# luchsonice/3dod

Hardware: AMD Instinct MI355X
Metric: images/sec Cube R-CNN DLA34-FPN train step (higher is better)
Workload: dtype fp32; 1 GPU; Cube R-CNN DLA34+FPN train step (fwd+loss+bwd+allreduce+SGD), 4 img/GPU 512x512, Base_Omni3D.yaml semantics (BASELINE configs[3] per-GPU shard); global_batch=4, parallelism=dp1, weight_gradient_reduce=pixel splits stored and added in a fixed order (CR_DETERMINISTIC=1), valid=True

## Files before the change

### 3dod_amd/_lib.py

```python
import ctypes
import os
import threading

import torch

_HERE = os.path.dirname(os.path.abspath(__file__))
LIB_PATH = os.path.join(_HERE, "lib", "libcr3dod.so")

c_void_p, c_int, c_int64, c_float = ctypes.c_void_p, ctypes.c_int, ctypes.c_int64, ctypes.c_float
P = c_void_p

SIGNATURES = {
    "cr_ctx_create": [c_int, P, ctypes.POINTER(P)],
    "cr_ctx_destroy": [P],
    "cr_ctx_set_stream": [P, P],
    "cr_abi_version": [],
    "cr_cuboid_corners": [P, P, P, c_int64, P],
    "cr_cubes_project_score": [P, P, c_int64, c_int64, P, c_int, c_float, c_float, P, P, P, P,
                               P, P, P, P, P, P, P, P, P],
    "cr_cubes_project_score_fast": [P, P, c_int64, c_int64, P, c_int, c_float, c_float, P, P, P, P,
                                    P, P, P, P, P, P, P, P, P, P],
    "cr_propose": [P, P, c_int64, P, c_int, c_int, P, P, P, c_int64, P, c_int, P, P, P, P, P],
    "cr_ransac_plane": [P, P, c_int64, P, c_int64, c_float, P, P, P],
    "cr_ransac_plane_batched": [P, P, P, c_int, c_int64, P, c_int64, c_float, P, P, P],
# ... 43 lines not shown
    "cr_conv2d_grouped_bwd_weight": [P, P, P, P, P, c_int, c_int, c_int, c_int, c_int, c_int, c_int, c_int, c_int, c_int, c_int,
                                     P, c_int64],
    "cr_cast_f32_to_bf16": [P, P, P, c_int64],
    "cr_weight_transpose": [P, P, P, c_int, c_int, c_int, c_int],
    "cr_colsum_accum": [P, P, c_int, c_int64, c_int, P, P],
    "cr_bn_fwd": [P, P, P, c_int, P, P, P, P, c_int64, c_int, c_int, c_float, c_float, P, P, P, c_int],
    "cr_bn_bwd": [P, P, P, P, P, P, P, P, P, P, P, c_int64, c_int, c_int, c_int],
    "cr_bn_bwd_mask": [P, P, P, P, P, P, P, P, P, P, P, P, c_int64, c_int, c_int, c_int],
    "cr_bn_frozen_unfold": [P, P, P, P, P, P, P, c_float, P, c_int, P, P, c_int, c_int],
    "cr_pool2x_fwd": [P, P, P, c_int, c_int, c_int, c_int, c_int, c_int],
    "cr_pool2x_bwd": [P, P, P, P, c_int, c_int, c_int, c_int, c_int, c_int, P],
    "cr_upsample2x_add": [P, P, P, P, c_int, c_int, c_int, c_int, c_int],
    "cr_sum2x2": [P, P, P, c_int, c_int, c_int, c_int, c_int],
    "cr_preprocess": [P, P, P, c_int, c_int, c_int, P, P, c_int],
    "cr_roi_align_fwd": [P, P, P, P, P, c_int, c_int, P, c_int64, c_int, c_int, P, c_int],
    "cr_roi_align_bwd": [P, P, P, P, P, c_int, c_int, P, c_int64, c_int, c_int, P, c_int],
    "cr_conv2d_fwd_group": [P, c_int, P, P, P, P, P, P, c_int, c_int, c_int, c_int, P, P, c_int, c_int],
    "cr_wino_filter": [P, P, P, c_int, c_int, c_int],
    "cr_gemm_batched_f32": [P, P, P, P, c_int, c_int, c_int, c_int, c_int64, c_int64, c_int64],
    "cr_wino_input": [P, c_int, P, P, P, P, c_int, P, c_int64],
    "cr_wino_output": [P, c_int, P, P, P, P, P, c_int, c_int64, P, c_int, P],
    "cr_wino_dy": [P, c_int, P, P, P, P, c_int, P, c_int64, P],
    "cr_wino_filter_grad": [P, P, P, c_int, c_int, P, P],
    "cr_wgrad_batched_f32": [P, P, P, P, c_int, c_int, c_int, c_int, c_int64, c_int64, c_int64],
    "cr_conv2d_bwd_data_group": [P, c_int, P, P, P, P, P, P, c_int, c_int, c_int, c_int, c_int, P],
    "cr_conv2d_bwd_weight_group": [P, c_int, P, P, P, P, P, P, P, c_int, c_int, c_int, c_int, c_int],
    "cr_conv2d_bwd_weight_multi": [P, c_int, P, P, P, P, P, P, P, P, P, P, P, P, c_int],
    "cr_roi_align_bwd_set": [P, P, P, P, P, c_int, c_int, c_int, P, c_int64, c_int, c_int, P, c_int],
    "cr_roi_pool_fwd": [P, P, P, P, P, c_int, c_int, c_int, P, c_int64, c_int, c_int, c_int, c_int, P, P, c_int],
    "cr_roi_pool_bwd": [P, P, P, P, P, c_int, c_int, c_int, P, c_int64, c_int, c_int, c_int, c_int, P, P, c_int],
    "cr_roi_pool_bwd_set": [P, P, P, P, P, c_int, c_int, c_int, P, c_int64, c_int, c_int, c_int, c_int, P, c_int],
    "cr_nms_grouped": [P, P, P, c_int, c_int, c_float, P, P],
    "cr_cube_loss_fwd": [P, P, c_int64, c_int, c_int, c_int, c_int, P, P],
    "cr_cube_loss_bwd": [P, P, c_int64, c_int, c_int, c_int, c_int, P, P, P, P, P, P],
    "cr_rpn_decode_select": [P, P, P, P, P, c_int, c_int, c_int, P, c_float, P, c_float, P, P, P],
    "cr_box_match": [P, P, c_int, P, P, c_int, c_int, c_int, P, P, P, P],
    "cr_rpn_label": [P, P, P, P, P, P, P, c_int, c_int, c_int, c_float, c_float, P, c_float, P, P, P, P],
    "cr_rpn_scatter": [P, P, P, c_int, P, P, c_int, c_int, P, c_float, c_int, c_int, P],
    "cr_rpn_loss": [P, P, P, P, P, P, P, c_int, c_int, c_int, P, P, P, P, P],
    "cr_rpn_loss_opt": [P, P, P, P, P, P, P, c_int, c_int, c_int, P, c_int, c_int, c_float, c_float, P, P, P, P],
    "cr_roi_label": [P, P, P, P, P, P, P, c_int, c_int, c_int, c_int, c_float, c_float, c_float, P, P, P],
    "cr_roi_compact": [P, P, P, c_int, P, P, c_int, c_int, P, P, P, c_int, c_int, P, P, P, P, P],
    "cr_box_loss": [P, P, P, P, P, P, P, P, c_int, c_int, c_int, c_int, P, c_float, P, P, P, P, P],
    "cr_box_loss_opt": [P, P, P, P, P, P, P, P, c_int, c_int, c_int, c_int, P, c_float, c_float, c_int, P, P, P, P, P],
    "cr_det_scores": [P, P, c_int, P, c_int, P, P, c_int, c_int, c_int, c_int, c_float, P, P],
    "cr_det_gather": [P, P, P, P, c_int, P, P, c_int, c_int, c_int, c_int, c_int, P, c_float, P, P, P, P],
# ... 165 lines not shown
```

### 3dod_amd/csrc/winograd.hip

```cpp
#include "cr_common.h"

#define WINO_MAX_MAPS 8
struct WinoMap { const float* src; float* dst; const float* acc; int N, H, W, tbase, blk0; };
struct WinoGeo { WinoMap m[WINO_MAX_MAPS]; int n, C, T; };

__device__ __forceinline__ int wino_find(const WinoGeo& g, int blk) {
    int i = 0;
    while (i + 1 < g.n && blk >= g.m[i + 1].blk0) ++i;
    return i;
}

typedef float vf1 __attribute__((ext_vector_type(1)));
typedef float vf2 __attribute__((ext_vector_type(2)));
typedef float vf4 __attribute__((ext_vector_type(4)));
#define WINO_TPB 8
#define WINO_TPB_DY 16
#define WINO_DB_SLOTS 16

struct WinoTile { int n, ty, tx, c; bool ok; };
template <int VEC>
__device__ __forceinline__ WinoTile wino_tile(const WinoGeo& g, const WinoMap& m, int tile_in_block, int tpb) {
    const int cgs = g.C / (64 * VEC);
    const int local = (int)blockIdx.x - m.blk0;
    const int cg = local % cgs, chunk = local / cgs;
// ... 59 lines not shown
            for (int e = 0; e < VEC; ++e) b[e] = bias[w.c + e];
        }
        const float* o = M + ((size_t)m.tbase + ((size_t)w.n * th + w.ty) * tw + w.tx) * C + w.c;
        VT q[4][4];
#pragma unroll
        for (int i = 0; i < 4; ++i)
#pragma unroll
            for (int j = 0; j < 4; ++j) q[i][j] = *(const VT*)(o + (i * 4 + j) * plane);
        VT s[2][4];
#pragma unroll
        for (int j = 0; j < 4; ++j) { s[0][j] = (q[0][j] + q[1][j]) + q[2][j]; s[1][j] = (q[1][j] - q[2][j]) - q[3][j]; }
#pragma unroll
        for (int i = 0; i < 2; ++i) {
            VT y0 = (s[i][0] + s[i][1]) + s[i][2] + b, y1 = (s[i][1] - s[i][2]) - s[i][3] + b;
            const size_t p = (((size_t)w.n * m.H + 2 * w.ty + i) * m.W + 2 * w.tx) * C + w.c;
            if (relu) { y0 = __builtin_elementwise_max(y0, (VT)(0.f)); y1 = __builtin_elementwise_max(y1, (VT)(0.f)); }
            if (m.acc) { y0 += *(const VT*)(m.acc + p); y1 += *(const VT*)(m.acc + p + C); }
            *(VT*)(m.dst + p) = y0;
            *(VT*)(m.dst + p + C) = y1;
        }
    }
}

__global__ __launch_bounds__(256) void k_wino_filter(const float* __restrict__ w, float* __restrict__ U, int O, int C, int mode) {
    const int idx = blockIdx.x * 256 + threadIdx.x;
    if (idx >= O * C) return;
    const int o = idx / C, c = idx - o * C;
    float g[3][3];
#pragma unroll
    for (int r = 0; r < 3; ++r)
#pragma unroll
        for (int s = 0; s < 3; ++s) g[r][s] = w[((size_t)(o * 3 + (mode ? 2 - r : r)) * 3 + (mode ? 2 - s : s)) * C + c];
    float t[4][3];
#pragma unroll
    for (int s = 0; s < 3; ++s) {
        t[0][s] = g[0][s];
        t[1][s] = 0.5f * ((g[0][s] + g[1][s]) + g[2][s]);
        t[2][s] = 0.5f * ((g[0][s] - g[1][s]) + g[2][s]);
        t[3][s] = g[2][s];
    }
    const size_t plane = (size_t)O * C;
    const size_t at = mode ? (size_t)c * O + o : (size_t)o * C + c;
#pragma unroll
    for (int i = 0; i < 4; ++i) {
        U[(i * 4 + 0) * plane + at] = t[i][0];
        U[(i * 4 + 1) * plane + at] = 0.5f * ((t[i][0] + t[i][1]) + t[i][2]);
        U[(i * 4 + 2) * plane + at] = 0.5f * ((t[i][0] - t[i][1]) + t[i][2]);
        U[(i * 4 + 3) * plane + at] = t[i][2];
    }
}

template <typename VT>
__global__ __launch_bounds__(256) void k_wino_dy(WinoGeo g, float* __restrict__ dM, float* __restrict__ db) {
    constexpr int VEC = sizeof(VT) / 4;
    __shared__ VT s_sum[4][64];
    const WinoMap& m = g.m[wino_find(g, (int)blockIdx.x)];
    const int C = g.C, th = m.H >> 1, tw = m.W >> 1;
    const int lane = threadIdx.x & 63, wave = threadIdx.x >> 6;
    const size_t plane = (size_t)g.T * C;
    VT acc = (VT)(0.f);
    int c = wino_tile<VEC>(g, m, 0, WINO_TPB_DY).c;
    for (int k = wave; k < WINO_TPB_DY; k += 4) {
        const WinoTile w = wino_tile<VEC>(g, m, k, WINO_TPB_DY);
        if (!w.ok) break;
        const float* p = m.src + (((size_t)w.n * m.H + 2 * w.ty) * m.W + 2 * w.tx) * C + w.c;
        const VT d00 = *(const VT*)p, d01 = *(const VT*)(p + C), d10 = *(const VT*)(p + (size_t)m.W * C),
                 d11 = *(const VT*)(p + (size_t)m.W * C + C);
        acc += (d00 + d01) + (d10 + d11);
        const VT t[4][2] = {{d00, d01}, {d00 + d10, d01 + d11}, {d00 - d10, d01 - d11}, {-d10, -d11}};
        float* o = dM + ((size_t)m.tbase + ((size_t)w.n * th + w.ty) * tw + w.tx) * C + w.c;
#pragma unroll
        for (int i = 0; i < 4; ++i) {
            *(VT*)(o + (i * 4 + 0) * plane) = t[i][0];
            *(VT*)(o + (i * 4 + 1) * plane) = t[i][0] + t[i][1];
            *(VT*)(o + (i * 4 + 2) * plane) = t[i][0] - t[i][1];
            *(VT*)(o + (i * 4 + 3) * plane) = -t[i][1];
        }
    }
    if (db) {
        s_sum[wave][lane] = acc;
        __syncthreads();
        if (wave == 0) {
            const VT v = (s_sum[0][lane] + s_sum[1][lane]) + (s_sum[2][lane] + s_sum[3][lane]);
#pragma unroll
            for (int e = 0; e < VEC; ++e) atomicAdd(db + (size_t)(blockIdx.x % WINO_DB_SLOTS) * C + c + e, v[e]);
        }
    }
}

__global__ __launch_bounds__(256) void k_wino_filter_grad(const float* __restrict__ dU, float* __restrict__ dw, int O, int C,
                                                          const float* __restrict__ db_part, float* __restrict__ db) {
    const int idx = blockIdx.x * 256 + threadIdx.x;
    if (idx >= O * C) return;
    const int o = idx / C, c = idx - o * C;
    if (db && c == 0) {
        float sum = 0.f;
        for (int k = 0; k < WINO_DB_SLOTS; ++k) sum += db_part[(size_t)k * O + o];
        db[o] += sum;
    }
    const size_t plane = (size_t)O * C;
    float u[4][4];
#pragma unroll
    for (int i = 0; i < 4; ++i)
#pragma unroll
        for (int j = 0; j < 4; ++j) u[i][j] = dU[(i * 4 + j) * plane + idx];
    float t[3][4];
#pragma unroll
    for (int j = 0; j < 4; ++j) {
        t[0][j] = u[0][j] + 0.5f * (u[1][j] + u[2][j]);
        t[1][j] = 0.5f * (u[1][j] - u[2][j]);
        t[2][j] = 0.5f * (u[1][j] + u[2][j]) + u[3][j];
    }
// ... 10 lines not shown
static int wino_geo(const char* who, WinoGeo& g, int n, const float* const* srcs, float* const* dsts, const float* const* accs,
                    const int* Ns, const int* Hs, const int* Ws, int C, int64_t T, int tpb, unsigned* blocks, int* vec) {
    CR_CHECK_ARG(n >= 1 && n <= WINO_MAX_MAPS, "%s: 1..%d maps", who, WINO_MAX_MAPS);
    CR_CHECK_ARG(C > 0 && C % 64 == 0, "%s: channels %% 64", who);
    g.n = n; g.C = C; g.T = (int)T;
    const int v = C % 256 == 0 ? 4 : C % 128 == 0 ? 2 : 1;
    *vec = v;
    int tb = 0, blk = 0;
    for (int i = 0; i < n; ++i) {
        CR_CHECK_ARG(Ns[i] > 0 && Hs[i] > 0 && Ws[i] > 0 && Hs[i] % 2 == 0 && Ws[i] % 2 == 0, "%s: map %d needs even H and W", who, i);
        g.m[i].src = srcs ? srcs[i] : nullptr; g.m[i].dst = dsts ? dsts[i] : nullptr; g.m[i].acc = accs ? accs[i] : nullptr;
        g.m[i].N = Ns[i]; g.m[i].H = Hs[i]; g.m[i].W = Ws[i]; g.m[i].tbase = tb; g.m[i].blk0 = blk;
        tb += Ns[i] * (Hs[i] / 2) * (Ws[i] / 2);
        blk += (int)cr_cdiv((int64_t)Ns[i] * (Hs[i] / 2) * (Ws[i] / 2), tpb) * (C / (64 * v));
    }
    CR_CHECK_ARG(tb == T && (int64_t)T * C * 16 < (1ll << 40), "%s: T = %lld does not match the maps (%d tiles)", who, (long long)T, tb);
    for (int i = n; i < WINO_MAX_MAPS; ++i) g.m[i] = g.m[n - 1];
    *blocks = (unsigned)blk;
    return CR_OK;
}

extern "C" int cr_wino_filter(cr_ctx* ctx, const float* w_krsc, float* U, int O, int C, int backward) {
    CR_CHECK_ARG(ctx && w_krsc && U && O > 0 && C > 0, "cr_wino_filter: bad args");
    hipLaunchKernelGGL(k_wino_filter, dim3((unsigned)cr_cdiv((int64_t)O * C, 256)), dim3(256), 0, ctx->stream, w_krsc, U, O, C, backward ? 1 : 0);
    CR_LAUNCH_CHECK();
    return CR_OK;
}

extern "C" int cr_wino_input(cr_ctx* ctx, int n, const float* const* xs, const int* Ns, const int* Hs, const int* Ws, int C,
                             float* V, int64_t T) {
    CR_CHECK_ARG(ctx && xs && Ns && Hs && Ws && V, "cr_wino_input: NULL pointer");
    WinoGeo g;
    unsigned blocks = 0;
    int vec = 1;
    int rc = wino_geo("cr_wino_input", g, n, xs, nullptr, nullptr, Ns, Hs, Ws, C, T, WINO_TPB, &blocks, &vec);
    if (rc) return rc;
    if (vec == 4) hipLaunchKernelGGL(k_wino_input<vf4>, dim3(blocks), dim3(256), 0, ctx->stream, g, V);
    else if (vec == 2) hipLaunchKernelGGL(k_wino_input<vf2>, dim3(blocks), dim3(256), 0, ctx->stream, g, V);
    else hipLaunchKernelGGL(k_wino_input<vf1>, dim3(blocks), dim3(256), 0, ctx->stream, g, V);
    CR_LAUNCH_CHECK();
    return CR_OK;
}

extern "C" int cr_wino_output(cr_ctx* ctx, int n, const float* M, float* const* ys, const int* Ns, const int* Hs, const int* Ws,
                              int O, int64_t T, const float* bias, int relu, const float* const* accs) {
    CR_CHECK_ARG(ctx && M && ys && Ns && Hs && Ws, "cr_wino_output: NULL pointer");
    WinoGeo g;
// ... 3 lines not shown
    if (rc) return rc;
    if (vec == 4) hipLaunchKernelGGL(k_wino_output<vf4>, dim3(blocks), dim3(256), 0, ctx->stream, g, M, bias, relu);
    else if (vec == 2) hipLaunchKernelGGL(k_wino_output<vf2>, dim3(blocks), dim3(256), 0, ctx->stream, g, M, bias, relu);
    else hipLaunchKernelGGL(k_wino_output<vf1>, dim3(blocks), dim3(256), 0, ctx->stream, g, M, bias, relu);
    CR_LAUNCH_CHECK();
    return CR_OK;
}

extern "C" int cr_wino_dy(cr_ctx* ctx, int n, const float* const* dys, const int* Ns, const int* Hs, const int* Ws, int O,
                          float* dM, int64_t T, float* db) {
    CR_CHECK_ARG(ctx && dys && Ns && Hs && Ws && dM, "cr_wino_dy: NULL pointer");
    WinoGeo g;
    unsigned blocks = 0;
    int vec = 1;
    int rc = wino_geo("cr_wino_dy", g, n, dys, nullptr, nullptr, Ns, Hs, Ws, O, T, WINO_TPB_DY, &blocks, &vec);
    if (rc) return rc;
    if (vec == 4) hipLaunchKernelGGL(k_wino_dy<vf4>, dim3(blocks), dim3(256), 0, ctx->stream, g, dM, db);
    else if (vec == 2) hipLaunchKernelGGL(k_wino_dy<vf2>, dim3(blocks), dim3(256), 0, ctx->stream, g, dM, db);
    else hipLaunchKernelGGL(k_wino_dy<vf1>, dim3(blocks), dim3(256), 0, ctx->stream, g, dM, db);
    CR_LAUNCH_CHECK();
    return CR_OK;
}

extern "C" int cr_wino_filter_grad(cr_ctx* ctx, const float* dU, float* dw, int O, int C, const float* db_part, float* db) {
    CR_CHECK_ARG(ctx && dU && dw && O > 0 && C > 0 && (!db == !db_part), "cr_wino_filter_grad: bad args");
    hipLaunchKernelGGL(k_wino_filter_grad, dim3((unsigned)cr_cdiv((int64_t)O * C, 256)), dim3(256), 0, ctx->stream, dU, dw, O, C,
                       db_part, db);
    CR_LAUNCH_CHECK();
    return CR_OK;
}
```

### 3dod_amd/cubercnn/modeling/graphed.py

```python
import contextlib
import gc

import torch
import torch.nn as nn

from ... import hipops as ops


@contextlib.contextmanager
def capture_guard():
    was = gc.isenabled()
    gc.collect()
    _empty_graveyard()
    gc.disable()
    keep, prev = [], ops._PLAN_KEEP[0]
    ops._PLAN_KEEP[0] = keep
    try:
        yield keep
    finally:
        ops._PLAN_KEEP[0] = prev
        if was:
            gc.enable()
        _empty_graveyard()

# ... 29 lines not shown
    dev = None

    def __del__(self):
        try:
            _bury_or_drain(self)
        except Exception:
            pass


@contextlib.contextmanager
def _fresh_leaves(modules):
    swapped = []
    for mod in modules:
        for m in mod.modules():
            for name, p in list(m._parameters.items()):
                if p is None:
                    continue
                q = nn.Parameter(p.data, requires_grad=p.requires_grad)
                sink = ops.grad_sink(p)
                if sink is not None:
                    q._cr_grad = sink
                if hasattr(p, "_cr_bank"):
                    q._cr_bank = p._cr_bank
                m._parameters[name] = q
                swapped.append((m, name, p))
    try:
        yield
    finally:
        for m, name, p in swapped:
            m._parameters[name] = p


class _Replay(torch.autograd.Function):
    @staticmethod
    def forward(ctx, runner, trigger):
        runner.fwd_graph.replay()
        ctx.runner = runner
        ctx.set_materialize_grads(False)
        return tuple(o.detach() for o in runner.static_outs)

    @staticmethod
    def backward(ctx, *grads):
        r = ctx.runner
        if r.pre_bwd is not None:
            r.pre_bwd()
        for sg, g in zip(r.static_grads, grads):
            if g is None:
                sg.zero_()
            elif g.data_ptr() != sg.data_ptr():
                sg.copy_(g)
        r.bwd_graph.replay()
        if r.bwd_graph2 is not None:
# ... 195 lines not shown
```

### 3dod_amd/hipops.py

```python
import contextlib
import ctypes
import math
import os

import torch

from . import _lib

bf16 = torch.bfloat16
f32 = torch.float32
STAT_REPL = 32

_PRECISIONS = {"fp32": (f32, 1), "f32": (f32, 1), "float32": (f32, 1), "fp32x3": (f32, 2), "bf16": (bf16, 0),
               "bfloat16": (bf16, 0)}
_ACT = [_PRECISIONS[os.environ.get("CR_PRECISION", "fp32").lower()]]


def set_precision(name):
    prev = precision()
    _ACT[0] = _PRECISIONS[str(name).lower()]
    return prev


def precision():
# ... 1022 lines not shown

def wino_supported(xs, weight, k, pad):
    return (winograd_on() and k == 3 and pad == 1 and xs[0].dtype == f32 and _ACT[0][1] == 1 and len(xs) <= 8
            and weight.shape[0] % 128 == 0 and weight.shape[1] % 128 == 0
            and all(x.shape[1] % 2 == 0 and x.shape[2] % 2 == 0 for x in xs))


WINO_MIN_TILES = int(os.environ.get("CR_WINO_MIN_TILES", "4096"))


def _wino_plan(xs, ws, bs, k, pad):
    n = len(xs)
    if not wino_supported(xs, ws[0], k, pad):
        return [False] * n
    if all(w is ws[0] for w in ws) and all(b is bs[0] for b in bs):
        return "shared"
    return [x.shape[0] * (x.shape[1] // 2) * (x.shape[2] // 2) >= WINO_MIN_TILES for x in xs]


def wino_gemm_raw(V, U, M, T, cin, cout):
    _lib.call("cr_gemm_batched_f32", V, U, M, T, cin, cout, 16, T * cin, cout * cin, T * cout)


def wino_conv3x3_group(srcs, w_krsc, dsts, bias, relu, accs, backward, keep_v=False):
    cast = lambda a: ctypes.cast(a, ctypes.c_void_p)
    assert w_krsc.dim() == 4 and w_krsc.shape[2:] == (3, 3) and w_krsc.is_contiguous(memory_format=torch.channels_last)
    O, C = w_krsc.shape[0], w_krsc.shape[1]
    cin, cout = (O, C) if backward else (C, O)
    dev = srcs[0].device
    T = sum(x.shape[0] * (x.shape[1] // 2) * (x.shape[2] // 2) for x in srcs)
    V, M, U = _wino_buffers(T, cin, cout, dev)
    U = U[:16 * O * C]
    if keep_v:
        V = torch.empty((16, T, cin), dtype=f32, device=dev)
    _lib.call("cr_wino_filter", w_krsc, U, O, C, int(backward))
    Ns, Hs, Ws = _int_table([x.shape[0] for x in srcs]), _int_table([x.shape[1] for x in srcs]), _int_table([x.shape[2] for x in srcs])
    _lib.call("cr_wino_input", len(srcs), cast(_ptr_table(srcs)), cast(Ns), cast(Hs), cast(Ws), cin, V, T)
    wino_gemm_raw(V, U, M, T, cin, cout)
    _lib.call("cr_wino_output", len(dsts), M, cast(_ptr_table(dsts)), cast(Ns), cast(Hs), cast(Ws), cout, T, bias, int(relu),
              cast(_ptr_table(accs)) if accs is not None else None)
    return V if keep_v else None


def wino_wgrad_on():
    return os.environ.get("CR_WINO_WGRAD", "1") != "0"


def deterministic_on():
    return os.environ.get("CR_DETERMINISTIC", "0") not in ("", "0")


def wino_wgrad_group(gs, xs, w_sink, b_sink, v_saved=None):
    cast = lambda a: ctypes.cast(a, ctypes.c_void_p)
    O, C = gs[0].shape[3], xs[0].shape[3]
    dev = xs[0].device
    T = sum(x.shape[0] * (x.shape[1] // 2) * (x.shape[2] // 2) for x in xs)
    V, M, U = _wino_buffers(T, C, O, dev)
    Ns, Hs, Ws = _int_table([x.shape[0] for x in xs]), _int_table([x.shape[1] for x in xs]), _int_table([x.shape[2] for x in xs])
    if v_saved is not None:
        assert v_saved.shape == (16, T, C)
        V = v_saved
    else:
        _lib.call("cr_wino_input", len(xs), cast(_ptr_table(xs)), cast(Ns), cast(Hs), cast(Ws), C, V, T)
    U.zero_()
    part = U[16 * O * C:] if b_sink is not None and not deterministic_on() else None
    if b_sink is not None and part is None:
        ws = torch.empty((1024, O), dtype=torch.float32, device=dev)
        for g in gs:
            _lib.call("cr_colsum_accum", g, 1, g.numel() // O, O, ws, b_sink)
    _lib.call("cr_wino_dy", len(gs), cast(_ptr_table(gs)), cast(Ns), cast(Hs), cast(Ws), O, M, T, part)
    _lib.call("cr_wgrad_batched_f32", M, V, U, T, C, O, 16, T * O, T * C, O * C)
    _lib.call("cr_wino_filter_grad", U, w_sink, O, C, part, b_sink if part is not None else None)


class _ConvBiasGroup(torch.autograd.Function):

    @staticmethod
    def forward(ctx, n, pad, relu, slots, *args):
        stacked = len(slots) == n + 1
        xs, ws, bs = args[:n], args[n:2 * n], args[2 * n:3 * n]
        Cout, Cin, k, _ = ws[0].shape
        dt = xs[0].dtype
        xs = [x.contiguous() for x in xs]
        wbs = [prepared_weights(w, False, dt)[0] for w in ws]
        shapes = [(x.shape[0], x.shape[1] + 2 * pad - k + 1, x.shape[2] + 2 * pad - k + 1, Cout) for x in xs]
        if stacked:
            rows = [s[0] * s[1] * s[2] for s in shapes]
            Y = torch.empty((1, 1, sum(rows), Cout), dtype=dt, device=xs[0].device)
            flat, off, ys = Y.view(-1, Cout), 0, []
            for s, m in zip(shapes, rows):
                ys.append(flat[off:off + m].view(s))
                off += m
        else:
            ys = [torch.empty(s, dtype=dt, device=x.device) for s, x in zip(shapes, xs)]
        bd = [None if b is None else b.detach() for b in bs]
        ctx.wino = plan = _wino_plan(xs, ws, bs, k, pad)
        keep = lambda i: (ctx.needs_input_grad[4 + n + i] and grad_sink(ws[i]) is not None and wino_wgrad_on()
                          and os.environ.get("CR_WINO_KEEP_V", "1") != "0")
        ctx.wino_v = {}
        if plan == "shared":
            ctx.wino_v["shared"] = wino_conv3x3_group(xs, wbs[0], ys, bd[0], relu, None, False, keep(0))
        else:
            for i in range(n):
                if plan[i]:
                    ctx.wino_v[i] = wino_conv3x3_group([xs[i]], wbs[i], [ys[i]], bd[i], relu, None, False, keep(i))
            rest = [i for i in range(n) if not plan[i]]
            if rest:
                conv_fwd_group_raw([xs[i] for i in rest], [wbs[i] for i in rest], [ys[i] for i in rest], Cin, Cout, k, pad,
                                   [bd[i] for i in rest], relu)
        ctx.cfg = (n, k, pad, relu)
        ctx.slots = slots
        ctx.refs = (ws, bs)
        ctx.stacked = shapes if stacked else None
        ctx.save_for_backward(*xs, *((Y,) if stacked and relu else (ys if relu else ())))
        ctx.set_materialize_grads(False)
        return Y if stacked else tuple(ys)

    @staticmethod
    def backward(ctx, *dys):
        n, k, pad, relu = ctx.cfg
        ws, bs = ctx.refs
        saved = ctx.saved_tensors
        xs = saved[:n]
        gs = {}
        if ctx.stacked is not None:
            live = list(range(n)) if dys[0] is not None else []
            if live:
                g = dys[0].contiguous()
                if relu:
                    g = relu_bwd(saved[n], g)
                g = g.to(xs[0].dtype).contiguous().view(-1, g.shape[-1])
                off = 0
                for i, s in enumerate(ctx.stacked):
                    m = s[0] * s[1] * s[2]
                    gs[i] = g[off:off + m].view(s)
                    off += m
        else:
            ys = saved[n:] if relu else (None,) * n
            live = [i for i in range(n) if dys[i] is not None]
            for i in live:
                g = dys[i].contiguous()
                if relu:
                    g = relu_bwd(ys[i], g)
                gs[i] = g.to(xs[i].dtype).contiguous()
        dt = xs[0].dtype
        Cout, Cin = ws[0].shape[0], ws[0].shape[1]
        dxs = [None] * n
        need_dx = [i for i in live if ctx.needs_input_grad[4 + i]]
        for i in range(n):
            if i not in need_dx and ctx.slots[i][0] is not None and i in live:
                raise RuntimeError("gradient slot registered for an input that needs no gradient")
        if need_dx:
            plan = ctx.wino
            outs = [torch.empty_like(xs[i]) for i in need_dx]
            accs = []
            for i in need_dx:
                slot, xi = ctx.slots[i]
                a = None if slot is None else (_slot_take(slot) if xi <= 1 else _slot_fold(slot))
                accs.append(None if a is None else a.to(dt).contiguous())
            if plan == "shared":
                wino_conv3x3_group([gs[i] for i in need_dx], prepared_weights(ws[0], False, dt)[0], outs, None, False, accs, True)
            else:
                for j, i in enumerate(need_dx):
                    if plan[i]:
                        wino_conv3x3_group([gs[i]], prepared_weights(ws[i], False, dt)[0], [outs[j]], None, False, [accs[j]], True)
                rest = [j for j, i in enumerate(need_dx) if not plan[i]]
                if rest:
                    conv_bwd_data_group_raw([gs[need_dx[j]] for j in rest], [prepared_weights(ws[need_dx[j]], True, dt)[1] for j in rest],
                                            [outs[j] for j in rest], [xs[need_dx[j]].shape for j in rest], Cin, Cout, k, pad,
                                            [accs[j] for j in rest])
            for i, o in zip(need_dx, outs):
                slot, xi = ctx.slots[i]
                if slot is not None and xi > 1:
                    _slot_put(slot, o)
                else:
                    dxs[i] = o
        dws, dbs = [None] * n, [None] * n
        wl = [i for i in live if ctx.needs_input_grad[4 + n + i]]
        sinks_ok = dt == f32 and all(grad_sink(ws[i]) is not None and (bs[i] is None or grad_sink(bs[i]) is not None) for i in wl)
        wplan = ctx.wino if sinks_ok and wino_wgrad_on() else None
        if wl and wplan == "shared":
            want_db = bs[0] is not None and ctx.needs_input_grad[4 + 2 * n + wl[0]]
            wino_wgrad_group([gs[i] for i in wl], [xs[i] for i in wl], grad_sink(ws[0]), grad_sink(bs[0]) if want_db else None,
                             ctx.wino_v.get("shared") if len(wl) == n else None)
            wl = []
        elif wl and wplan is not None and any(wplan[i] for i in wl):
            for i in [i for i in wl if wplan[i]]:
                want_db = bs[i] is not None and ctx.needs_input_grad[4 + 2 * n + i]
                wino_wgrad_group([gs[i]], [xs[i]], grad_sink(ws[i]), grad_sink(bs[i]) if want_db else None, ctx.wino_v.get(i))
            wl = [i for i in wl if not wplan[i]]
        if wl and sinks_ok and len(wl) > 1:
            dwt = [grad_sink(ws[i]) for i in wl]
            dbt = [None if bs[i] is None or not ctx.needs_input_grad[4 + 2 * n + i] else grad_sink(bs[i]) for i in wl]
            conv_bwd_weight_group_raw([gs[i] for i in wl], [xs[i] for i in wl], dwt, dbt, Cin, Cout, k, pad)
        else:
            for i in wl:
                bsink = None if bs[i] is None else grad_sink(bs[i])
                want_db = bs[i] is not None and ctx.needs_input_grad[4 + 2 * n + i]
                acc = None
                if want_db:
                    acc = bsink if bsink is not None else torch.zeros((Cout,), dtype=f32, device=xs[i].device)
                    if bsink is None:
                        dbs[i] = acc if dbs[i] is None else dbs[i] + acc
                dws[i] = conv_bwd_weight_raw(gs[i], xs[i], k, 1, pad, grad_sink(ws[i]), bias_acc=acc)
        return (None, None, None, None) + tuple(dxs) + tuple(dws) + tuple(dbs)


def conv_bias_act_group(xs, weights, biases, pad=0, relu=False, stacked=False):
    xs, weights, biases = list(xs), [as_krsc(w) for w in weights], list(biases)
    if not group_supported(xs, weights):
# ... 2136 lines not shown
```

### include/cr3dod.h

```cpp
#ifndef CR3DOD_H
#define CR3DOD_H

#include <stdint.h>

#ifdef __cplusplus
extern "C" {
#endif

typedef struct cr_ctx cr_ctx;

#define CR_OK 0
#define CR_EINVAL (-22)
#define CR_ENOMEM (-12)
#define CR_EHIP (-5)
#define CR_ERANGE (-34)

int cr_ctx_create(int device, void* hip_stream, cr_ctx** out);
int cr_ctx_destroy(cr_ctx* ctx);
int cr_ctx_set_stream(cr_ctx* ctx, void* hip_stream);
const char* cr_last_error(void);
int cr_abi_version(void);


int cr_cuboid_corners(cr_ctx* ctx, const float* box6, const float* R, int64_t n, float* verts);
// ... 102 lines not shown
               const float* const* boxes3d_ptrs, const float* const* poses_ptrs, const int* counts, int B, int G,
               float* boxes, int64_t* classes, float* boxes3d, float* poses);
int cr_topk_blocks(int64_t n, int k);
int cr_topk(cr_ctx* ctx, const float* x, int rows, int64_t n, int k, void* ws, float* vals, int64_t* idx);
int cr_loss_guard(cr_ctx* ctx, const float* vals, int n, float scale, float* red, float* total, float* recent,
                  int stabilize, float tolerance, float gamma, int* flag);
int cr_step_counters(cr_ctx* ctx, const int* flag, float* explode, float* success);
int cr_multi_seg(cr_ctx* ctx, const void* descs_dev, int ndesc, int64_t total, int accumulate);
int cr_relu_bwd(cr_ctx* ctx, const void* y, const void* dy, void* g, int64_t n, int act_f32);
int cr_fold_bn(cr_ctx* ctx, const float* w, const float* gamma, const float* beta, const float* mean, const float* var,
               float eps, void* wf, float* bias, int Cout, int K, int act_f32);

int cr_conv2d_bwd_weight_bias(cr_ctx* ctx, const void* dy, const void* x, float* dw, float* dbias, int N, int H, int W,
                              int Cin, int Cout, int ks, int stride, int pad, int accumulate, int act_f32);
int cr_conv2d_grouped_fwd(cr_ctx* ctx, const void* x, const float* w, void* y, int N, int H, int W, int Cin, int Cout,
                          int groups, int ks, int stride, int pad, const float* bias, const void* residual, int relu,
                          float* stats, int act_f32);
int cr_conv2d_grouped_bwd_data(cr_ctx* ctx, const void* dy, const float* w, void* dx, int N, int H, int W, int Cin,
                               int Cout, int groups, int ks, int stride, int pad, int act_f32, const void* accumulate);
int cr_conv2d_grouped_bwd_weight(cr_ctx* ctx, const void* dy, const void* x, float* dw, float* dbias, int N, int H, int W,
                                 int Cin, int Cout, int groups, int ks, int stride, int pad, int accumulate, int act_f32,
                                 float* ws, int64_t ws_floats);
int cr_wino_filter(cr_ctx* ctx, const float* w_krsc, float* U, int O, int C, int backward);
int cr_gemm_batched_f32(cr_ctx* ctx, const float* x, const float* w, float* y, int R, int K, int O, int batches,
                        int64_t stride_x, int64_t stride_w, int64_t stride_y);
int cr_wino_input(cr_ctx* ctx, int n, const float* const* xs, const int* Ns, const int* Hs, const int* Ws, int C,
                  float* V, int64_t T);
int cr_wino_output(cr_ctx* ctx, int n, const float* M, float* const* ys, const int* Ns, const int* Hs, const int* Ws,
                   int O, int64_t T, const float* bias, int relu, const float* const* accs);
int cr_wino_dy(cr_ctx* ctx, int n, const float* const* dys, const int* Ns, const int* Hs, const int* Ws, int O,
               float* dM, int64_t T, float* db_part);
int cr_wino_filter_grad(cr_ctx* ctx, const float* dU, float* dw, int O, int C, const float* db_part, float* db);
int cr_wgrad_batched_f32(cr_ctx* ctx, const float* dy, const float* x, float* dw, int R, int K, int O, int batches,
                         int64_t stride_dy, int64_t stride_x, int64_t stride_dw);

int cr_conv2d_fwd_group(cr_ctx* ctx, int n, const void* const* xs, const void* const* ws, void* const* ys, const int* Ns,
                        const int* Hs, const int* Ws, int Cin, int Cout, int ks, int pad, const float* const* biases,
                        const void* const* residuals, int relu, int act_f32);
int cr_conv2d_bwd_data_group(cr_ctx* ctx, int n, const void* const* dys, const void* const* wts, void* const* dxs,
                             const int* Ns, const int* Hs, const int* Ws, int Cin, int Cout, int ks, int pad, int act_f32,
                             const void* const* accumulates);
int cr_conv2d_bwd_weight_group(cr_ctx* ctx, int n, const void* const* dys, const void* const* xs, float* const* dws,
                               float* const* dbiases, const int* Ns, const int* Hs, const int* Ws, int Cin, int Cout, int ks,
                               int pad, int act_f32);
int cr_conv2d_bwd_weight_multi(cr_ctx* ctx, int n, const void* const* dys, const void* const* xs, float* const* dws,
                               float* const* dbiases, const int* Ns, const int* Hs, const int* Ws, const int* Cins,
                               const int* Couts, const int* kss, const int* strides, const int* pads, int act_f32);
int cr_cast_f32_to_bf16(cr_ctx* ctx, const float* src, void* dst, int64_t n);
int cr_colsum_accum(cr_ctx* ctx, const void* x, int is_f32, int64_t M, int C, float* ws, float* out);
int cr_weight_transpose(cr_ctx* ctx, const float* w, void* wt, int Cout, int ks, int Cin, int act_f32);

int cr_bn_fwd(cr_ctx* ctx, const void* x, const float* stats, int nparts, const float* gamma, const float* beta,
              const void* residual, void* y, int64_t M, int C, int relu, float eps, float momentum,
              float* mean_invstd, float* running_mean, float* running_var, int act_f32);
int cr_bn_bwd(cr_ctx* ctx, const void* dy, const void* out, const void* x, const float* mean_invstd,
// ... 260 lines not shown
```

Before: 247.6 images/s.

## Fuse Winograd backward dy transforms with ReLU mask and cache filter transforms

Adds a fused kernel that reads the output gradient once, applies the ReLU mask from the saved output, and writes both the data-grad Winograd input tiles and the weight-grad dM tiles with nontemporal stores, replacing separate relu_bwd, wino_input and wino_dy passes. Forward and backward filter transforms are now computed together in one kernel and cached per weight version, so repeated transforms across forward, backward and graph replays are skipped. Cache state is carried across the graphed parameter swap. This adds complexity and a per-weight buffer, and the cached transform must be allocated before graph capture.

New measurement: 246.7 images/s. About the same (-0.3%).

```diff
diff --git a/3dod_amd/_lib.py b/3dod_amd/_lib.py
--- a/3dod_amd/_lib.py
+++ b/3dod_amd/_lib.py
@@ -89,6 +89,8 @@
     "cr_wino_output": [P, c_int, P, P, P, P, P, c_int, c_int64, P, c_int, P],
     "cr_wino_dy": [P, c_int, P, P, P, P, c_int, P, c_int64, P],
     "cr_wino_filter_grad": [P, P, P, c_int, c_int, P, P],
+    "cr_wino_filter_pair": [P, P, P, P, c_int, c_int],
+    "cr_wino_grad": [P, c_int, P, P, P, P, P, c_int, P, P, c_int64, P],
     "cr_wgrad_batched_f32": [P, P, P, P, c_int, c_int, c_int, c_int, c_int64, c_int64, c_int64],
     "cr_conv2d_bwd_data_group": [P, c_int, P, P, P, P, P, P, c_int, c_int, c_int, c_int, c_int, P],
     "cr_conv2d_bwd_weight_group": [P, c_int, P, P, P, P, P, P, P, c_int, c_int, c_int, c_int, c_int],
diff --git a/3dod_amd/csrc/winograd.hip b/3dod_amd/csrc/winograd.hip
--- a/3dod_amd/csrc/winograd.hip
+++ b/3dod_amd/csrc/winograd.hip
@@ -105,15 +105,7 @@
     }
 }
 
-__global__ __launch_bounds__(256) void k_wino_filter(const float* __restrict__ w, float* __restrict__ U, int O, int C, int mode) {
-    const int idx = blockIdx.x * 256 + threadIdx.x;
-    if (idx >= O * C) return;
-    const int o = idx / C, c = idx - o * C;
-    float g[3][3];
-#pragma unroll
-    for (int r = 0; r < 3; ++r)
-#pragma unroll
-        for (int s = 0; s < 3; ++s) g[r][s] = w[((size_t)(o * 3 + (mode ? 2 - r : r)) * 3 + (mode ? 2 - s : s)) * C + c];
+__device__ __forceinline__ void wino_filter_store(const float (&g)[3][3], float* __restrict__ U, size_t plane, size_t at) {
     float t[4][3];
 #pragma unroll
     for (int s = 0; s < 3; ++s) {
@@ -122,14 +114,34 @@
         t[2][s] = 0.5f * ((g[0][s] - g[1][s]) + g[2][s]);
         t[3][s] = g[2][s];
     }
-    const size_t plane = (size_t)O * C;
-    const size_t at = mode ? (size_t)c * O + o : (size_t)o * C + c;
 #pragma unroll
     for (int i = 0; i < 4; ++i) {
         U[(i * 4 + 0) * plane + at] = t[i][0];
         U[(i * 4 + 1) * plane + at] = 0.5f * ((t[i][0] + t[i][1]) + t[i][2]);
         U[(i * 4 + 2) * plane + at] = 0.5f * ((t[i][0] - t[i][1]) + t[i][2]);
         U[(i * 4 + 3) * plane + at] = t[i][2];
+    }
+}
+
+__global__ __launch_bounds__(256) void k_wino_filter(const float* __restrict__ w, float* __restrict__ Uf, float* __restrict__ Ub,
+                                                     int O, int C) {
+    const int idx = blockIdx.x * 256 + threadIdx.x;
+    if (idx >= O * C) return;
+    const int o = idx / C, c = idx - o * C;
+    float g[3][3];
+#pragma unroll
+    for (int r = 0; r < 3; ++r)
+#pragma unroll
+        for (int s = 0; s < 3; ++s) g[r][s] = w[((size_t)(o * 3 + r) * 3 + s) * C + c];
+    const size_t plane = (size_t)O * C;
+    if (Uf) wino_filter_store(g, Uf, plane, (size_t)o * C + c);
+    if (Ub) {
+        float h[3][3];
+#pragma unroll
+        for (int r = 0; r < 3; ++r)
+#pragma unroll
+            for (int s = 0; s < 3; ++s) h[r][s] = g[2 - r][2 - s];
+        wino_filter_store(h, Ub, plane, (size_t)c * O + o);
     }
 }
 
@@ -171,6 +183,87 @@
     }
 }
 
+#define WINO_ST(p, v) __builtin_nontemporal_store((v), (p))
+template <typename VT, bool MASKED, bool WANT_V>
+__device__ __forceinline__ void wino_grad_window(const WinoMap& m, const WinoTile& w, int C, VT (&d)[4][4]) {
+    constexpr int VEC = sizeof(VT) / 4;
+#pragma unroll
+    for (int i = 0; i < 4; ++i) {
+        const int y = 2 * w.ty - 1 + i, yc = min(max(y, 0), m.H - 1);
+#pragma unroll
+        for (int j = 0; j < 4; ++j) {
+            if (!WANT_V && !((i == 1 || i == 2) && (j == 1 || j == 2))) { d[i][j] = (VT)(0.f); continue; }
+            const int x = 2 * w.tx - 1 + j, xc = min(max(x, 0), m.W - 1);
+            const size_t at = (((size_t)w.n * m.H + yc) * m.W + xc) * C + w.c;
+            VT v = *(const VT*)(m.src + at);
+            if (MASKED) {
+                const VT a = *(const VT*)(m.acc + at);
+#pragma unroll
+                for (int e = 0; e < VEC; ++e) v[e] = a[e] > 0.f ? v[e] : 0.f;
+            }
+            d[i][j] = ((unsigned)y < (unsigned)m.H && (unsigned)x < (unsigned)m.W) ? v : (VT)(0.f);
+        }
+    }
+}
+
+template <typename VT, bool WANT_V>
+__global__ __launch_bounds__(256) void k_wino_grad(WinoGeo g, float* __restrict__ V, float* __restrict__ dM, float* __restrict__ db) {
+    constexpr int VEC = sizeof(VT) / 4;
+    __shared__ VT s_sum[4][64];
+    const WinoMap& m = g.m[wino_find(g, (int)blockIdx.x)];
+    const int C = g.C, th = m.H >> 1, tw = m.W >> 1;
+    const int lane = threadIdx.x & 63, wave = threadIdx.x >> 6;
+    const size_t plane = (size_t)g.T * C;
+    VT acc = (VT)(0.f);
+    const int c = wino_tile<VEC>(g, m, 0, WINO_TPB_DY).c;
+    for (int k = wave; k < WINO_TPB_DY; k += 4) {
+        const WinoTile w = wino_tile<VEC>(g, m, k, WINO_TPB_DY);
+        if (!w.ok) break;
+        VT d[4][4];
+        if (m.acc) wino_grad_window<VT, true, WANT_V>(m, w, C, d);
+        else wino_grad_window<VT, false, WANT_V>(m, w, C, d);
+        const size_t row = ((size_t)m.tbase + ((size_t)w.n * th + w.ty) * tw + w.tx) * C + w.c;
+        if (WANT_V) {
+            VT t[4][4];
+#pragma unroll
+            for (int j = 0; j < 4; ++j) {
+                t[0][j] = d[0][j] - d[2][j]; t[1][j] = d[1][j] + d[2][j]; t[2][j] = d[2][j] - d[1][j]; t[3][j] = d[1][j] - d[3][j];
+            }
+            float* o = V + row;
+#pragma unroll
+            for (int i = 0; i < 4; ++i) {
+                WINO_ST((VT*)(o + (i * 4 + 0) * plane), t[i][0] - t[i][2]);
+                WINO_ST((VT*)(o + (i * 4 + 1) * plane), t[i][1] + t[i][2]);
+                WINO_ST((VT*)(o + (i * 4 + 2) * plane), t[i][2] - t[i][1]);
+                WINO_ST((VT*)(o + (i * 4 + 3) * plane), t[i][1] - t[i][3]);
+            }
+        }
+        if (dM) {
+            const VT d00 = d[1][1], d01 = d[1][2], d10 = d[2][1], d11 = d[2][2];
+            acc += (d00 + d01) + (d10 + d11);
+            const VT t[4][2] = {{d00, d01}, {d00 + d10, d01 + d11}, {d00 - d10, d01 - d11}, {-d10, -d11}};
+            float* o = dM + row;
+#pragma unroll
+            for (int i = 0; i < 4; ++i) {
+                WINO_ST((VT*)(o + (i * 4 + 0) * plane), t[i][0]);
+                WINO_ST((VT*)(o + (i * 4 + 1) * plane), t[i][0] + t[i][1]);
+                WINO_ST((VT*)(o + (i * 4 + 2) * plane), t[i][0] - t[i][1]);
+                WINO_ST((VT*)(o + (i * 4 + 3) * plane), -t[i][1]);
+            }
+        }
+    }
+    if (db) {
+        s_sum[wave][lane] = acc;
+        __syncthreads();
+        if (wave == 0) {
+            const VT v = (s_sum[0][lane] + s_sum[1][lane]) + (s_sum[2][lane] + s_sum[3][lane]);
+#pragma unroll
+            for (int e = 0; e < VEC; ++e) atomicAdd(db + (size_t)(blockIdx.x % WINO_DB_SLOTS) * C + c + e, v[e]);
+        }
+    }
+}
+#undef WINO_ST
+
 __global__ __launch_bounds__(256) void k_wino_filter_grad(const float* __restrict__ dU, float* __restrict__ dw, int O, int C,
                                                           const float* __restrict__ db_part, float* __restrict__ db) {
     const int idx = blockIdx.x * 256 + threadIdx.x;
@@ -227,7 +320,15 @@
 
 extern "C" int cr_wino_filter(cr_ctx* ctx, const float* w_krsc, float* U, int O, int C, int backward) {
     CR_CHECK_ARG(ctx && w_krsc && U && O > 0 && C > 0, "cr_wino_filter: bad args");
-    hipLaunchKernelGGL(k_wino_filter, dim3((unsigned)cr_cdiv((int64_t)O * C, 256)), dim3(256), 0, ctx->stream, w_krsc, U, O, C, backward ? 1 : 0);
+    hipLaunchKernelGGL(k_wino_filter, dim3((unsigned)cr_cdiv((int64_t)O * C, 256)), dim3(256), 0, ctx->stream, w_krsc,
+                       backward ? nullptr : U, backward ? U : nullptr, O, C);
+    CR_LAUNCH_CHECK();
+    return CR_OK;
+}
+
+extern "C" int cr_wino_filter_pair(cr_ctx* ctx, const float* w_krsc, float* U_fwd, float* U_bwd, int O, int C) {
+    CR_CHECK_ARG(ctx && w_krsc && U_fwd && U_bwd && U_fwd != U_bwd && O > 0 && C > 0, "cr_wino_filter_pair: bad args");
+    hipLaunchKernelGGL(k_wino_filter, dim3((unsigned)cr_cdiv((int64_t)O * C, 256)), dim3(256), 0, ctx->stream, w_krsc, U_fwd, U_bwd, O, C);
     CR_LAUNCH_CHECK();
     return CR_OK;
 }
@@ -277,6 +378,28 @@
     return CR_OK;
 }
 
+extern "C" int cr_wino_grad(cr_ctx* ctx, int n, const float* const* dys, const float* const* ys, const int* Ns, const int* Hs,
+                            const int* Ws, int O, float* V, float* dM, int64_t T, float* db) {
+    CR_CHECK_ARG(ctx && dys && Ns && Hs && Ws && (V || dM) && V != dM && (!db || dM), "cr_wino_grad: bad args");
+    WinoGeo g;
+    unsigned blocks = 0;
+    int vec = 1;
+    int rc = wino_geo("cr_wino_grad", g, n, dys, nullptr, ys, Ns, Hs, Ws, O, T, WINO_TPB_DY, &blocks, &vec);
+    if (rc) return rc;
+    for (int i = 0; i < n; ++i) CR_CHECK_ARG(dys[i], "cr_wino_grad: map %d is NULL", i);
+#define WINO_GRAD_LAUNCH(VT)                                                                                          \
+    do {                                                                                                              \
+        if (V) hipLaunchKernelGGL((k_wino_grad<VT, true>), dim3(blocks), dim3(256), 0, ctx->stream, g, V, dM, db);      \
+        else hipLaunchKernelGGL((k_wino_grad<VT, false>), dim3(blocks), dim3(256), 0, ctx->stream, g, V, dM, db);       \
+    } while (0)
+    if (vec == 4) WINO_GRAD_LAUNCH(vf4);
+    else if (vec == 2) WINO_GRAD_LAUNCH(vf2);
+    else WINO_GRAD_LAUNCH(vf1);
+#undef WINO_GRAD_LAUNCH
+    CR_LAUNCH_CHECK();
+    return CR_OK;
+}
+
 extern "C" int cr_wino_filter_grad(cr_ctx* ctx, const float* dU, float* dw, int O, int C, const float* db_part, float* db) {
     CR_CHECK_ARG(ctx && dU && dw && O > 0 && C > 0 && (!db == !db_part), "cr_wino_filter_grad: bad args");
     hipLaunchKernelGGL(k_wino_filter_grad, dim3((unsigned)cr_cdiv((int64_t)O * C, 256)), dim3(256), 0, ctx->stream, dU, dw, O, C,
diff --git a/3dod_amd/cubercnn/modeling/graphed.py b/3dod_amd/cubercnn/modeling/graphed.py
--- a/3dod_amd/cubercnn/modeling/graphed.py
+++ b/3dod_amd/cubercnn/modeling/graphed.py
@@ -75,12 +75,17 @@
                     q._cr_grad = sink
                 if hasattr(p, "_cr_bank"):
                     q._cr_bank = p._cr_bank
+                if hasattr(p, "_cr_wino_u"):
+                    q._cr_wino_u = p._cr_wino_u
                 m._parameters[name] = q
                 swapped.append((m, name, p))
     try:
         yield
     finally:
         for m, name, p in swapped:
+            q = m._parameters[name]
+            if hasattr(q, "_cr_wino_u"):
+                p._cr_wino_u = q._cr_wino_u
             m._parameters[name] = p
 
 
diff --git a/3dod_amd/hipops.py b/3dod_amd/hipops.py
--- a/3dod_amd/hipops.py
+++ b/3dod_amd/hipops.py
@@ -1068,7 +1068,29 @@
     _lib.call("cr_gemm_batched_f32", V, U, M, T, cin, cout, 16, T * cin, cout * cin, T * cout)
 
 
-def wino_conv3x3_group(srcs, w_krsc, dsts, bias, relu, accs, backward, keep_v=False):
+def wino_fused_grad_on():
+    return os.environ.get("CR_WINO_FUSED_GRAD", "1") != "0"
+
+
+def wino_filter_pair(weight):
+    O, C = weight.shape[0], weight.shape[1]
+    tag = (weight._version, _WEIGHT_EPOCH[0], weight.data_ptr())
+    ent = getattr(weight, "_cr_wino_u", None)
+    if ent is None or ent[1].device != weight.device or ent[1].shape != (2, 16, O * C):
+        if weight.is_cuda and torch.cuda.is_current_stream_capturing():
+            raise _lib.CrError("winograd: the transformed filters must be allocated before the graph capture (run one eager pass first)")
+        ent = [None, torch.empty((2, 16, O * C), dtype=f32, device=weight.device)]
+        try:
+            weight._cr_wino_u = ent
+        except Exception:
+            pass
+    if ent[0] != tag:
+        _lib.call("cr_wino_filter_pair", weight.detach(), ent[1][0], ent[1][1], O, C)
+        ent[0] = tag
+    return ent[1][0], ent[1][1]
+
+
+def wino_conv3x3_group(srcs, w_krsc, dsts, bias, relu, accs, backward, keep_v=False, owner=None):
     cast = lambda a: ctypes.cast(a, ctypes.c_void_p)
     assert w_krsc.dim() == 4 and w_krsc.shape[2:] == (3, 3) and w_krsc.is_contiguous(memory_format=torch.channels_last)
     O, C = w_krsc.shape[0], w_krsc.shape[1]
@@ -1076,10 +1098,13 @@
     dev = srcs[0].device
     T = sum(x.shape[0] * (x.shape[1] // 2) * (x.shape[2] // 2) for x in srcs)
     V, M, U = _wino_buffers(T, cin, cout, dev)
-    U = U[:16 * O * C]
     if keep_v:
         V = torch.empty((16, T, cin), dtype=f32, device=dev)
-    _lib.call("cr_wino_filter", w_krsc, U, O, C, int(backward))
+    if owner is not None and owner.data_ptr() == w_krsc.data_ptr():
+        U = wino_filter_pair(owner)[int(bool(backward))]
+    else:
+        U = U[:16 * O * C]
+        _lib.call("cr_wino_filter", w_krsc, U, O, C, int(backward))
     Ns, Hs, Ws = _int_table([x.shape[0] for x in srcs]), _int_table([x.shape[1] for x in srcs]), _int_table([x.shape[2] for x in srcs])
     _lib.call("cr_wino_input", len(srcs), cast(_ptr_table(srcs)), cast(Ns), cast(Hs), cast(Ws), cin, V, T)
     wino_gemm_raw(V, U, M, T, cin, cout)
@@ -1117,6 +1142,31 @@
     _lib.call("cr_wino_dy", len(gs), cast(_ptr_table(gs)), cast(Ns), cast(Hs), cast(Ws), O, M, T, part)
     _lib.call("cr_wgrad_batched_f32", M, V, U, T, C, O, 16, T * O, T * C, O * C)
     _lib.call("cr_wino_filter_grad", U, w_sink, O, C, part, b_sink if part is not None else None)
+
+
+def wino_grad_group(gs, ys, weight, w_sink, b_sink, v_saved, outs, accs, colsum_gs=None):
+    cast = lambda a: ctypes.cast(a, ctypes.c_void_p)
+    O, C = weight.shape[0], weight.shape[1]
+    dev = gs[0].device
+    T = sum(g.shape[0] * (g.shape[1] // 2) * (g.shape[2] // 2) for g in gs)
+    assert v_saved.shape == (16, T, C)
+    Vg, Mx, _ = _wino_buffers(T, O, C, dev) if outs is not None else (None, None, None)
+    _, M, U = _wino_buffers(T, C, O, dev)
+    Ns, Hs, Ws = _int_table([g.shape[0] for g in gs]), _int_table([g.shape[1] for g in gs]), _int_table([g.shape[2] for g in gs])
+    U.zero_()
+    part = U[16 * O * C:] if b_sink is not None and not deterministic_on() else None
+    if b_sink is not None and part is None:
+        ws = torch.empty((1024, O), dtype=torch.float32, device=dev)
+        for g in colsum_gs:
+            _lib.call("cr_colsum_accum", g, 1, g.numel() // O, O, ws, b_sink)
+    _lib.call("cr_wino_grad", len(gs), cast(_ptr_table(gs)), cast(_ptr_table(ys)) if ys is not None else None, cast(Ns), cast(Hs),
+              cast(Ws), O, Vg, M, T, part)
+    _lib.call("cr_wgrad_batched_f32", M, v_saved, U, T, C, O, 16, T * O, T * C, O * C)
+    _lib.call("cr_wino_filter_grad", U, w_sink, O, C, part, b_sink if part is not None else None)
+    if outs is not None:
+        wino_gemm_raw(Vg, wino_filter_pair(weight)[1], Mx, T, O, C)
+        _lib.call("cr_wino_output", len(outs), Mx, cast(_ptr_table(outs)), cast(Ns), cast(Hs), cast(Ws), C, T, None, 0,
+                  cast(_ptr_table(accs)) if accs is not None else None)
 
 
 class _ConvBiasGroup(torch.autograd.Function):
@@ -1145,11 +1195,11 @@
                           and os.environ.get("CR_WINO_KEEP_V", "1") != "0")
         ctx.wino_v = {}
         if plan == "shared":
-            ctx.wino_v["shared"] = wino_conv3x3_group(xs, wbs[0], ys, bd[0], relu, None, False, keep(0))
+            ctx.wino_v["shared"] = wino_conv3x3_group(xs, wbs[0], ys, bd[0], relu, None, False, keep(0), owner=ws[0])
         else:
             for i in range(n):
                 if plan[i]:
-                    ctx.wino_v[i] = wino_conv3x3_group([xs[i]], wbs[i], [ys[i]], bd[i], relu, None, False, keep(i))
+                    ctx.wino_v[i] = wino_conv3x3_group([xs[i]], wbs[i], [ys[i]], bd[i], relu, None, False, keep(i), owner=ws[i])
             rest = [i for i in range(n) if not plan[i]]
             if rest:
                 conv_fwd_group_raw([xs[i] for i in rest], [wbs[i] for i in rest], [ys[i] for i in rest], Cin, Cout, k, pad,
@@ -1168,48 +1218,79 @@
         ws, bs = ctx.refs
         saved = ctx.saved_tensors
         xs = saved[:n]
-        gs = {}
+        dt = xs[0].dtype
+        Cout, Cin = ws[0].shape[0], ws[0].shape[1]
+        plan = ctx.wino
         if ctx.stacked is not None:
             live = list(range(n)) if dys[0] is not None else []
+        else:
+            live = [i for i in range(n) if dys[i] is not None]
+        need_dx = [i for i in live if ctx.needs_input_grad[4 + i]]
+        for i in range(n):
+            if i not in need_dx and ctx.slots[i][0] is not None and i in live:
+                raise RuntimeError("gradient slot registered for an input that needs no gradient")
+        wl = [i for i in live if ctx.needs_input_grad[4 + n + i]]
+        sinks_ok = dt == f32 and all(grad_sink(ws[i]) is not None and (bs[i] is None or grad_sink(bs[i]) is not None) for i in wl)
+        wplan = plan if sinks_ok and wino_wgrad_on() else None
+        fused = {}
+        if wino_fused_grad_on() and wl and wplan == "shared":
+            if len(wl) == n and ctx.wino_v.get("shared") is not None and (need_dx == wl or not need_dx):
+                fused["shared"] = wl
+        elif wino_fused_grad_on() and wl and wplan is not None:
+            fused = {i: [i] for i in wl if wplan[i] and ctx.wino_v.get(i) is not None}
+        gs, ymaps, colsum_gs = {}, None, None
+        if ctx.stacked is not None:
             if live:
                 g = dys[0].contiguous()
-                if relu:
+                if relu and "shared" in fused:
+                    y = saved[n].view(-1, g.shape[-1])
+                    want_db = bs[0] is not None and ctx.needs_input_grad[4 + 2 * n + wl[0]]
+                    gm = relu_bwd(saved[n], g).view(-1, g.shape[-1]) if want_db and deterministic_on() else None
+                    ymaps, colsum_gs = [], ([] if gm is not None else None)
+                elif relu:
                     g = relu_bwd(saved[n], g)
                 g = g.to(xs[0].dtype).contiguous().view(-1, g.shape[-1])
                 off = 0
                 for i, s in enumerate(ctx.stacked):
                     m = s[0] * s[1] * s[2]
                     gs[i] = g[off:off + m].view(s)
+                    if ymaps is not None:
+                        ymaps.append(y[off:off + m].view(s))
+                        if colsum_gs is not None:
+                            colsum_gs.append(gm[off:off + m].view(s))
                     off += m
         else:
             ys = saved[n:] if relu else (None,) * n
-            live = [i for i in range(n) if dys[i] is not None]
             for i in live:
                 g = dys[i].contiguous()
                 if relu:
                     g = relu_bwd(ys[i], g)
                 gs[i] = g.to(xs[i].dtype).contiguous()
-        dt = xs[0].dtype
-        Cout, Cin = ws[0].shape[0], ws[0].shape[1]
         dxs = [None] * n
-        need_dx = [i for i in live if ctx.needs_input_grad[4 + i]]
-        for i in range(n):
-            if i not in need_dx and ctx.slots[i][0] is not None and i in live:
-                raise RuntimeError("gradient slot registered for an input that needs no gradient")
+        outs, accs = [], []
         if need_dx:
-            plan = ctx.wino
             outs = [torch.empty_like(xs[i]) for i in need_dx]
-            accs = []
             for i in need_dx:
                 slot, xi = ctx.slots[i]
                 a = None if slot is None else (_slot_take(slot) if xi <= 1 else _slot_fold(slot))
                 accs.append(None if a is None else a.to(dt).contiguous())
+        for key, maps in fused.items():
+            want_db = bs[maps[0]] is not None and ctx.needs_input_grad[4 + 2 * n + maps[0]]
+            js = [need_dx.index(i) for i in maps if i in need_dx]
+            mg = [gs[i] for i in maps]
+            wino_grad_group(mg, ymaps, ws[maps[0]], grad_sink(ws[maps[0]]), grad_sink(bs[maps[0]]) if want_db else None,
+                            ctx.wino_v[key], [outs[j] for j in js] if js else None, [accs[j] for j in js] if js else None,
+                            colsum_gs if colsum_gs is not None else mg)
+        if need_dx:
             if plan == "shared":
-                wino_conv3x3_group([gs[i] for i in need_dx], prepared_weights(ws[0], False, dt)[0], outs, None, False, accs, True)
+                if "shared" not in fused:
+                    wino_conv3x3_group([gs[i] for i in need_dx], prepared_weights(ws[0], False, dt)[0], outs, None, False, accs, True,
+                                       owner=ws[0])
             else:
                 for j, i in enumerate(need_dx):
-                    if plan[i]:
-                        wino_conv3x3_group([gs[i]], prepared_weights(ws[i], False, dt)[0], [outs[j]], None, False, [accs[j]], True)
+                    if plan[i] and i not in fused:
+                        wino_conv3x3_group([gs[i]], prepared_weights(ws[i], False, dt)[0], [outs[j]], None, False, [accs[j]], True,
+                                           owner=ws[i])
                 rest = [j for j, i in enumerate(need_dx) if not plan[i]]
                 if rest:
                     conv_bwd_data_group_raw([gs[need_dx[j]] for j in rest], [prepared_weights(ws[need_dx[j]], True, dt)[1] for j in rest],
@@ -1222,16 +1303,14 @@
                 else:
                     dxs[i] = o
         dws, dbs = [None] * n, [None] * n
-        wl = [i for i in live if ctx.needs_input_grad[4 + n + i]]
-        sinks_ok = dt == f32 and all(grad_sink(ws[i]) is not None and (bs[i] is None or grad_sink(bs[i]) is not None) for i in wl)
-        wplan = ctx.wino if sinks_ok and wino_wgrad_on() else None
         if wl and wplan == "shared":
-            want_db = bs[0] is not None and ctx.needs_input_grad[4 + 2 * n + wl[0]]
-            wino_wgrad_group([gs[i] for i in wl], [xs[i] for i in wl], grad_sink(ws[0]), grad_sink(bs[0]) if want_db else None,
-                             ctx.wino_v.get("shared") if len(wl) == n else None)
+            if "shared" not in fused:
+                want_db = bs[0] is not None and ctx.needs_input_grad[4 + 2 * n + wl[0]]
+                wino_wgrad_group([gs[i] for i in wl], [xs[i] for i in wl], grad_sink(ws[0]), grad_sink(bs[0]) if want_db else None,
+                                 ctx.wino_v.get("shared") if len(wl) == n else None)
             wl = []
         elif wl and wplan is not None and any(wplan[i] for i in wl):
-            for i in [i for i in wl if wplan[i]]:
+            for i in [i for i in wl if wplan[i] and i not in fused]:
                 want_db = bs[i] is not None and ctx.needs_input_grad[4 + 2 * n + i]
                 wino_wgrad_group([gs[i]], [xs[i]], grad_sink(ws[i]), grad_sink(bs[i]) if want_db else None, ctx.wino_v.get(i))
             wl = [i for i in wl if not wplan[i]]
diff --git a/include/cr3dod.h b/include/cr3dod.h
--- a/include/cr3dod.h
+++ b/include/cr3dod.h
@@ -148,6 +148,7 @@
                                  int Cin, int Cout, int groups, int ks, int stride, int pad, int accumulate, int act_f32,
                                  float* ws, int64_t ws_floats);
 int cr_wino_filter(cr_ctx* ctx, const float* w_krsc, float* U, int O, int C, int backward);
+int cr_wino_filter_pair(cr_ctx* ctx, const float* w_krsc, float* U_fwd, float* U_bwd, int O, int C);
 int cr_gemm_batched_f32(cr_ctx* ctx, const float* x, const float* w, float* y, int R, int K, int O, int batches,
                         int64_t stride_x, int64_t stride_w, int64_t stride_y);
 int cr_wino_input(cr_ctx* ctx, int n, const float* const* xs, const int* Ns, const int* Hs, const int* Ws, int C,
@@ -157,6 +158,8 @@
 int cr_wino_dy(cr_ctx* ctx, int n, const float* const* dys, const int* Ns, const int* Hs, const int* Ws, int O,
                float* dM, int64_t T, float* db_part);
 int cr_wino_filter_grad(cr_ctx* ctx, const float* dU, float* dw, int O, int C, const float* db_part, float* db);
+int cr_wino_grad(cr_ctx* ctx, int n, const float* const* dys, const float* const* ys, const int* Ns, const int* Hs,
+                 const int* Ws, int O, float* V, float* dM, int64_t T, float* db_part);
 int cr_wgrad_batched_f32(cr_ctx* ctx, const float* dy, const float* x, float* dw, int R, int K, int O, int batches,
                          int64_t stride_dy, int64_t stride_x, int64_t stride_dw);
 
```
